# laurentbartholdi/SpaSM.jl

Measured on AMD Instinct MI355X. Metric: Schur nnz reduced/sec (GF(p) echelonize), 1Mx1M CSR, higher is better.
Workload: dtype int32 (GF(p) balanced residues); 1 GPU; BASELINE config 3: 1000000x1000000 CSR, 20 nnz/row, p=65521, seed 0x5A5A0003, Schur round 0; rows_per_gpu=1000000, npiv=169473, nnz_out=522630694, parallelism=single GPU

## Files before the change

### spasm.jl_amd/csrc/engine.hip

```cpp
#include "common.hpp"
#include "kernels.hpp"
#include "stream.hpp"
#include "wlevel.hpp"
#include "greedy.hpp"
#include "dense.hpp"
#include "spmv.hpp"
#include "spgemm.hpp"
#include "reshape.hpp"
#include "trsolve.hpp"
#include "batch.hpp"
#include "blocks.hpp"
#include "solve_batch.hpp"
#include "solver.hpp"
#include <cstring>
#include <rocprim/device/device_scan.hpp>
#include <rocprim/device/device_radix_sort.hpp>
#include <rocprim/device/device_segmented_radix_sort.hpp>
#include <vector>
#include <memory>
#include <stdexcept>
#include <type_traits>
#include <algorithm>
#include <cstring>
#include <cstdlib>
// ... 1311 lines not shown
    {
        if (bigsc_m == m) return;
        const i64 per = std::max<i64>((i64)m, 1) * 13;
        bigsc_blocks = (int)std::max<i64>(1, std::min<i64>((i64)num_cu * 8, ((i64)2 << 30) / per));
        bigsc_m = m;
        const size_t nw = ((size_t)std::max(m, 1) + 31) / 32;
        sc_xdense.alloc((size_t)bigsc_blocks * (size_t)std::max(m, 1));
        sc_bitmap.alloc((size_t)bigsc_blocks * nw);
        sc_touched.alloc((size_t)bigsc_blocks * (size_t)std::max(m, 1));
        sc_xdense.zero(s);
        sc_bitmap.zero(s);
    }
    void warm_scatter()
    {
        ensure_streams();
        ensure_big_scatter(stream);
        ScatterArgs a;
        memset(&a, 0, sizeof a);
        StreamArgs sa;
        memset(&sa, 0, sizeof sa);
        const int nhash = F.small ? kNumHashClasses : kNumHashClasses - 1;
        for (int c = 0; c < nhash; c++) {
            const size_t lds = scatter_lds_bytes(kClasses[c], F.small);
            if (F.small) launch_scatter_class<true>(c, a, 0, lds, stream);
            else launch_scatter_class<false>(c, a, 0, lds, stream);
        }
        for (int c = 0; c < std::min(nhash, kNumStreamClasses); c++) {
            const size_t lds = stream_lds_bytes(stream_logt(c), stream_tpr(c), stream_wpb(c));
            const StreamMode mode = stream_mode(use_w ? wbase + wcap : 0);
            if (F.small) launch_stream_class<true>(c, sa, 0, num_cu, lds, stream, mode);
            else launch_stream_class<false>(c, sa, 0, num_cu, lds, stream, mode);
        }
    }

    void run_scatter(const DevMat &M, const int *rows, int nrows)
    {
        const int4 *recs = Lpool.p;
        S.n = nrows;
        S.m = m;
        nlaunch = 0;
        if (nrows == 0) return;
        int nhash = F.small ? kNumHashClasses : kNumHashClasses - 1;
        const bool streaming = use_w && !force_lists && !want_idx;
        BinArgs b;
        b.nrows = nrows;
        b.bound = bound.p;
        b.Llen = Llen.p;
        for (int c = 0; c < NCLASS; c++) b.cap[c] = -1;
        for (int c = 0; c < nhash; c++) b.cap[c] = kClasses[c].cap;
        b.lazy_terms = zp_lazy_terms(F);
        b.class_count = class_count.p;
        b.class_list = class_list.p;
        b.rows = rows;
        b.start = M.start.p;
        b.len = M.len.p;
        b.orig = M.orig.p;
        b.Lstart = Lstart.p;
        b.sstart = sstart.p;
        b.pmask = pmask.p;
        b.sflag = sflag.p;
        b.stream_classes = streaming ? std::min(nhash, kNumStreamClasses) : 0;
        b.Sorig = S.orig.p;
        b.fixcnt = fixcnt.p;
        b.desc = class_desc.p;
        hipLaunchKernelGGL(k_bin, dim3(cdiv(nrows, 1024)), dim3(256), 0, stream, b);
        HIPCHK(hipGetLastError());

        ScatterArgs a;
        a.ent = M.ent.p;
        a.qinv_r = qinv_r.p;
        a.uhdr = uhdr.p;
        a.UPN = UPN.p;
        a.Lpool = recs;
        a.Sent = S.ent.p;
        a.Slen = S.len.p;
        a.Slead = S.lead.p;
        a.ctr = ctr.p;
        a.F = F;
        {
            const char *dbg = getenv("SPASM_DBG");
            a.dbg = dbg ? atoi(dbg) : 0;
        }
        a.stamps = nullptr;
#ifdef SPASM_STAMPS
        stamps.ensure(NCLASS * 2 * NSTAMP);
        HIPCHK(hipMemsetAsync(stamps.p, 0, NCLASS * 2 * NSTAMP * sizeof(u64d), stream));
        a.stamps = stamps.p;
#endif
        StreamArgs sa;
        sa.ent = M.ent.p;
        sa.qinv_r = qinv_r.p;
        sa.UPN = UPN.p;
        sa.Lpool = recs;
        sa.Sent = S.ent.p;
        sa.Slen = S.len.p;
        sa.Slead = S.lead.p;
        sa.ctr = ctr.p;
        sa.F = F;
        sa.dbg = a.dbg;
        sa.stamps = a.stamps;
        sa.fixbuf = fixbuf.p;
        sa.fixcnt = fixcnt.p;
        nhash_used = nhash;
        const int first_side = 6;
        const bool use_side = !class_timing && (nhash > first_side || streaming);
        if (use_side) {
            ensure_streams();
            HIPCHK(hipEventRecord(ev_fork, stream));
            HIPCHK(hipStreamWaitEvent(side, ev_fork, 0));
        }
        auto mark = [&](int cls_id, hipStream_t s) {
            if (!class_timing || nlaunch >= NCLASS) return;
            HIPCHK(hipEventRecord(ev_cls[nlaunch], s));
            launch_cls[nlaunch++] = cls_id;
        };
        auto launch_class = [&](int c, hipStream_t s) {
            mark(c, s);
            a.cls = c;
            a.class_count = class_count.p + c;
            a.desc = class_desc.p + (size_t)c * nrows;
            const size_t lds = scatter_lds_bytes(kClasses[c], F.small);
            int per_cu = (int)std::min<size_t>(32 / kClasses[c].wpb, (160 * 1024) / lds);
            if (per_cu < 1) per_cu = 1;
            const int rows_per_block = kClasses[c].tpr == 64 ? kClasses[c].wpb : 1;
            const int grid = std::max(1, std::min(cdiv(nrows, rows_per_block), num_cu * per_cu));
            if (F.small) launch_scatter_class<true>(c, a, grid, lds, s);
            else launch_scatter_class<false>(c, a, grid, lds, s);
        };
        auto launch_stream_cls = [&](int c, hipStream_t s) {
            if (!streaming || c >= kNumStreamClasses) return;
            mark(NSTREAM0 + c, s);
            sa.cls = NSTREAM0 + c;
            sa.class_count = class_count.p + NSTREAM0 + c;
            sa.desc = class_desc.p + (size_t)(NSTREAM0 + c) * nrows;
            sa.redo_count = class_count.p + c;
            sa.redo_desc = class_desc.p + (size_t)c * nrows;
            const size_t lds = stream_lds_bytes(stream_logt(c), stream_tpr(c), stream_wpb(c));
            if (F.small) launch_stream_class<true>(c, sa, nrows, num_cu, lds, s, smode);
            else launch_stream_class<false>(c, sa, nrows, num_cu, lds, s, smode);
        };
        auto launch_stream_fix = [&](hipStream_t s) {
            if (!streaming) return;
            mark(NCLASS - 1, s);
            StreamFixArgs fa;
            fa.nrows = nrows;
            fa.fixcnt = fixcnt.p;
            fa.fixbuf = fixbuf.p;
            fa.sstart = sstart.p;
            fa.Sent = S.ent.p;
            fa.Slen = S.len.p;
            fa.Slead = S.lead.p;
            fa.ctr = ctr.p;
            fa.F = F;
            hipLaunchKernelGGL(k_stream_fix, dim3(cdiv(nrows, 64)), dim3(256), 0, s, fa);
            HIPCHK(hipGetLastError());
        };
        auto launch_big = [&](hipStream_t s) {
            ensure_big_scatter(s);
            mark(NHASHMAX - 1, s);
            BigScatterArgs bb;
            bb.s = a;
            bb.s.cls = NHASHMAX - 1;
            bb.s.class_count = class_count.p + (NHASHMAX - 1);
            bb.s.desc = class_desc.p + (size_t)(NHASHMAX - 1) * nrows;
            bb.m = std::max(m, 1);
            bb.nwords = (std::max(m, 1) + 31) / 32;
            bb.xdense = sc_xdense.p;
            bb.bitmap = sc_bitmap.p;
            bb.touched = sc_touched.p;
            hipLaunchKernelGGL(k_scatter_big, dim3(bigsc_blocks), dim3(256), 0, s, bb);
            HIPCHK(hipGetLastError());
        };
        if (use_side && streaming) {
            const int lanes = n_lanes();
            for (int l = 1; l < lanes; l++) HIPCHK(hipStreamWaitEvent(lane_s[l], ev_fork, 0));
            const int ntwin = n_twins();
            for (int c = nhash - 1; c >= 0; c--) {
                const int l = (nhash - 1 - c) % lanes;
                hipStream_t lane = l ? lane_s[l] : stream;
                launch_stream_cls(c, lane);
                HIPCHK(hipEventRecord(ev_cls_done[c], lane));
                const int t = (nhash - 1 - c) % ntwin;
                hipStream_t tw = t ? twin_s[t - 1] : side;
                HIPCHK(hipStreamWaitEvent(tw, ev_cls_done[c], 0));
                launch_class(c, tw);
            }
            for (int l = 1; l < lanes; l++) {
                HIPCHK(hipEventRecord(lane_ev[l], lane_s[l]));
                HIPCHK(hipStreamWaitEvent(stream, lane_ev[l], 0));
            }
            for (int t = 0; t < ntwin - 1; t++) {
                HIPCHK(hipEventRecord(twin_ev[t], twin_s[t]));
                HIPCHK(hipStreamWaitEvent(stream, twin_ev[t], 0));
            }
            launch_stream_fix(stream);
            launch_big(side);
            HIPCHK(hipEventRecord(ev_join, side));
            HIPCHK(hipStreamWaitEvent(stream, ev_join, 0));
        } else if (use_side) {
            for (int c = nhash - 1; c >= first_side; c--) launch_class(c, side);
            launch_big(side);
            HIPCHK(hipEventRecord(ev_join, side));
            for (int c = 0; c < first_side; c++) launch_class(c, stream);
            HIPCHK(hipStreamWaitEvent(stream, ev_join, 0));
        } else {
            for (int c = nhash - 1; c >= 0; c--) launch_stream_cls(c, stream);
            launch_stream_fix(stream);
            for (int c = 0; c < nhash; c++) launch_class(c, stream);
            launch_big(stream);
            if (class_timing) HIPCHK(hipEventRecord(ev_cls[nlaunch], stream));
        }
        hipLaunchKernelGGL(k_scatter_mark_failed, dim3(cdiv(nrows, 256)), dim3(256), 0, stream, nrows, Llen.p, S.len.p, S.lead.p);
        HIPCHK(hipGetLastError());
        HIPCHK(hipMemcpyAsync(S.start.p, sstart.p, ((size_t)nrows + 1) * sizeof(i64d), hipMemcpyDeviceToDevice, stream));
    }

    void fetch_counters()
    {
        hctr = read_counters();
        int *cc = hclass_count;
        HIPCHK(hipMemcpyAsync(cc, class_count.p, NCLASS * sizeof(int), hipMemcpyDeviceToHost, stream));
        HIPCHK(hipStreamSynchronize(stream));
#ifdef SPASM_STAMPS
        {
            std::vector<u64d> h(NCLASS * 2 * NSTAMP);
            HIPCHK(hipMemcpy(h.data(), stamps.p, h.size() * sizeof(u64d), hipMemcpyDeviceToHost));
            static const char *names[NSTAMP] = {"prologue", "issue", "wait-loads", "own", "rounds", "remainder", "sweep", "-"};
            static const char *snames[NSTAMP] = {"top+own", "chunks", "next-req", "rowend", "reset", "rotate", "-", "-"};
            for (int c = NSTREAM0; c < NCLASS; c++) {
                const double waves = (double)h[(size_t)c * 2 * NSTAMP + NSTAMP];
                if (waves == 0) continue;
                fprintf(stderr, "[stamps] stream class %d rows %d waves %.0f: cycles per wave:", c - NSTREAM0, cc[c], waves);
                for (int i = 0; i < 6; i++) fprintf(stderr, " %s=%.0f", snames[i], (double)h[(size_t)c * 2 * NSTAMP + i] / waves);
                fprintf(stderr, "\n");
            }
            for (int c = 0; c < NHASHMAX; c++) {
                const double waves = (double)h[(size_t)c * 2 * NSTAMP + NSTAMP];
                if (waves == 0) continue;
                fprintf(stderr, "[stamps] class %d rows %d waves %.0f: cycles per wave:", c, cc[c], waves);
                for (int i = 0; i < 7; i++) fprintf(stderr, " %s=%.0f", names[i], (double)h[(size_t)c * 2 * NSTAMP + i] / waves);
                fprintf(stderr, "\n");
            }
        }
#endif
        if (hctr.lpool_overflow) throw EngineError("multiplier pool exhausted");
        if (hctr.scatter_overflow) throw EngineError("a hash table of the scatter kernel filled up (internal bound violated)");
    }
};

void upload_csr_strided(const struct spasm_csr *A, int row_lo, int row_hi, int stride, DevMat &M, hipStream_t s);

void upload_csr(const struct spasm_csr *A, int row_lo, int row_hi, DevMat &M, hipStream_t s)
{
    const int n = row_hi - row_lo;
    const i64 base = A->p[row_lo];
    const i64 nnz = A->p[row_hi] - base;
    M.n = n;
    M.m = A->m;
    M.start.ensure((size_t)n + 1);
    M.len.ensure((size_t)n + 1);
    M.lead.ensure((size_t)n + 1);
    M.orig.ensure((size_t)n + 1);
    M.ent.ensure((size_t)nnz + 1);
    DevBuf<i64d> dp;
    DevBuf<int> dj, dx;
    dp.alloc((size_t)n + 1);
    dj.alloc((size_t)nnz + 1);
    dx.alloc((size_t)nnz + 1);
    std::vector<i64d> hp((size_t)n + 1);
    for (int i = 0; i <= n; i++) hp[(size_t)i] = A->p[row_lo + i] - base;
    HIPCHK(hipMemcpyAsync(dp.p, hp.data(), ((size_t)n + 1) * sizeof(i64d), hipMemcpyHostToDevice, s));
    if (nnz > 0) {
        HIPCHK(hipMemcpyAsync(dj.p, A->j + base, (size_t)nnz * sizeof(int), hipMemcpyHostToDevice, s));
        if (A->x) HIPCHK(hipMemcpyAsync(dx.p, A->x + base, (size_t)nnz * sizeof(int), hipMemcpyHostToDevice, s));
        hipLaunchKernelGGL(k_pack_entries, dim3(std::min<i64>(cdiv(nnz, 256), 65536)), dim3(256), 0, s, (i64d)nnz, zp_field_make(A->field->p), dj.p,
                           A->x ? dx.p : nullptr, M.ent.p);
        HIPCHK(hipGetLastError());
    }
    if (n > 0) {
        hipLaunchKernelGGL(k_pack_rows, dim3(cdiv(n, 256)), dim3(256), 0, s, n, row_lo, 1, dp.p, M.start.p, M.len.p, M.orig.p);
        HIPCHK(hipGetLastError());
        constexpr int TEAM = 8;
        if (A->x) hipLaunchKernelGGL((k_drop_zeros<TEAM>), dim3(cdiv((i64)n * TEAM, 256)), dim3(256), 0, s, n, M.start.p, M.len.p, M.ent.p);
        hipLaunchKernelGGL((k_row_lead<TEAM>), dim3(cdiv((i64)n * TEAM, 256)), dim3(256), 0, s, n, M.start.p, M.len.p, M.ent.p, M.lead.p);
        HIPCHK(hipGetLastError());
    }
    HIPCHK(hipStreamSynchronize(s));
}

void upload_csr_strided(const struct spasm_csr *A, int row_lo, int row_hi, int stride, DevMat &M, hipStream_t s)
{
    if (stride <= 1) { upload_csr(A, row_lo, row_hi, M, s); return; }
    const int n = row_hi > row_lo ? (row_hi - row_lo + stride - 1) / stride : 0;
    std::vector<i64d> hp((size_t)n + 1, 0);
    for (int i = 0; i < n; i++) { const int g = row_lo + i * stride; hp[(size_t)i + 1] = hp[(size_t)i] + (A->p[g + 1] - A->p[g]); }
    const i64 nnz = hp[(size_t)n];
    std::vector<int> hj((size_t)nnz + 1), hx((size_t)nnz + 1);
    for (int i = 0; i < n; i++) {
        const int g = row_lo + i * stride;
        const i64 len = A->p[g + 1] - A->p[g];
        memcpy(hj.data() + hp[(size_t)i], A->j + A->p[g], sizeof(int) * (size_t)len);
        if (A->x) memcpy(hx.data() + hp[(size_t)i], A->x + A->p[g], sizeof(int) * (size_t)len);
    }
    M.n = n;
    M.m = A->m;
    M.start.ensure((size_t)n + 1);
    M.len.ensure((size_t)n + 1);
// ... 7615 lines not shown
```

### spasm.jl_amd/csrc/stream.hpp

```cpp
#pragma once
#include "kernels.hpp"

struct StreamArgs {
    const int *class_count;
    const RowDesc *desc;
    const int2 *ent;
    const int *qinv_r;
    const int2 *UPN;
    const int4 *Lpool;
    int2 *Sent;
    int *Slen;
    int *Slead;
    RoundCounters *ctr;
    int cls;
    int *redo_count;
    RowDesc *redo_desc;
    int2 *fixbuf;
    int *fixcnt;
    u64d *stamps;
    int dbg;
    ZpField F;
};

constexpr int SLCAP = 64;
constexpr int SFIX = 64;

__host__ __device__ constexpr size_t stream_row_bytes(int logt) { return ((size_t)7 << logt) + 64 + (size_t)SFIX * 8 + (size_t)SLCAP * 16; }
__host__ __device__ constexpr size_t stream_lds_bytes(int logt, int tpr, int wpb) { return tpr == 64 ? stream_row_bytes(logt) * (size_t)wpb : stream_row_bytes(logt); }

__device__ __forceinline__ void stream_fix_push(int *s_nfix, int2 *fix, int fcap, int owner_pos, int pos, int v)
{
    const int i = atomicAdd(s_nfix, 1);
    if (i < fcap) fix[i] = make_int2((int)(((unsigned)owner_pos << 14) | (unsigned)pos), v);
}

constexpr unsigned STREAM_K1 = 0x9E3779u, STREAM_K2 = 0x85EBCBu, STREAM_K3 = 0xC2B2AFu;

template <bool SMALL> __device__ __forceinline__ int stream_mul(const ZpField &F, int nm, int y);
template <> __device__ __forceinline__ int stream_mul<true>(const ZpField &F, int nm, int y) { return acc_reduce_short<true>(F, __mul24(nm, y)); }
template <> __device__ __forceinline__ int stream_mul<false>(const ZpField &F, int nm, int y) { return zp_mul(F, nm, y); }

__device__ __forceinline__ u64d stream_load_fresh(const u64d *p) { return __hip_atomic_load(p, __ATOMIC_RELAXED, __HIP_MEMORY_SCOPE_AGENT); }

template <int FCAP>
__device__ __forceinline__ int stream_fixup(const ZpField F, const int2 *fix, int nfix, int *scratch, u64d *row, int E, int *lead)
{
    constexpr int HC = 2 * FCAP;
    const int lane = threadIdx.x & 63;
    int *holes = scratch, *tailflag = scratch + HC, *lowh = scratch + 2 * HC, *livet = scratch + 3 * HC;
    for (int b = 0; b < nfix; b += 64) {
        const int f = b + lane;
        if (f < nfix) {
            const int2 e = fix[f];
            const int po = (int)((unsigned)e.x >> 14);
            holes[f] = e.x & 0x3fff;
            u64d *p = row + po;
            u64d cur = stream_load_fresh(p);
            for (;;) {
                const int nv = zp_add(F, (int)(cur >> 32), e.y);
                const u64d want = ((u64d)(unsigned)nv << 32) | (cur & 0xffffffffull);
                const u64d old = atomicCAS(p, cur, want);
                if (old == cur) break;
                cur = old;
            }
        }
    }
    int nh = nfix, nz = 0;
    for (int b = 0; b < nfix; b += 64) {
        const int f = b + lane;
        int po = -1;
        bool z = false;
        if (f < nfix) {
            po = (int)((unsigned)fix[f].x >> 14);
            z = (int)(stream_load_fresh(row + po) >> 32) == 0;
        }
        u64d mz = __ballot(z);
        while (mz) {
            const int l = __ffsll((long long)mz) - 1;
            mz &= mz - 1;
            const int pz = __shfl(po, l);
            bool dup = false;
            for (int i = nfix + lane; i < nh; i += 64) dup |= holes[i] == pz;
            if (__ballot(dup) == 0) {
                if (lane == 0) holes[nh] = pz;
                nh++;
                nz++;
            }
        }
    }
    const int n_out = E - nh;
    for (int i = lane; i < nh; i += 64) tailflag[i] = 0;
    for (int i = lane; i < nh; i += 64) {
        const int hp = holes[i];
        if (hp >= n_out) tailflag[hp - n_out] = 1;
    }
    int nlow = 0, nlive = 0;
    for (int b = 0; b < nh; b += 64) {
        const int i = b + lane;
        const bool in = i < nh;
        const int hp = in ? holes[i] : INT_MAX;
        const bool low = in && hp < n_out;
        const u64d ml = __ballot(low);
        if (low) lowh[nlow + __popcll(ml & lanemask_lt())] = hp;
        nlow += __popcll(ml);
        const bool live = in && tailflag[i] == 0;
        const u64d mv = __ballot(live);
        if (live) livet[nlive + __popcll(mv & lanemask_lt())] = n_out + i;
        nlive += __popcll(mv);
    }
    for (int i = lane; i < nlow; i += 64) row[lowh[i]] = stream_load_fresh(row + livet[i]);
    if (nz > 0) {
        asm volatile("s_waitcnt vmcnt(0)" ::: "memory");
        int mn = INT_MAX;
        for (int i = lane; i < n_out; i += 64) mn = min(mn, (int)(unsigned)stream_load_fresh(row + i));
        *lead = wave_min_i32(mn);
    }
    return n_out;
}


__device__ __forceinline__ int stream_desc_load(const RowDesc *p) { return ((const int *)p)[(threadIdx.x & 63) % 12]; }
__device__ __forceinline__ RowDesc stream_desc_unpack(int v)
{
    RowDesc d;
    const unsigned w0 = __builtin_amdgcn_readlane(v, 0), w1 = __builtin_amdgcn_readlane(v, 1), w2 = __builtin_amdgcn_readlane(v, 2),
                   w3 = __builtin_amdgcn_readlane(v, 3), w4 = __builtin_amdgcn_readlane(v, 4), w5 = __builtin_amdgcn_readlane(v, 5),
                   w10 = __builtin_amdgcn_readlane(v, 10), w11 = __builtin_amdgcn_readlane(v, 11);
    d.ent_start = (i64d)(((u64d)w1 << 32) | w0);
    d.l_start = (i64d)(((u64d)w3 << 32) | w2);
    d.s_start = (i64d)(((u64d)w5 << 32) | w4);
    d.len = __builtin_amdgcn_readlane(v, 6);
    d.llen = __builtin_amdgcn_readlane(v, 7);
    d.t = __builtin_amdgcn_readlane(v, 8);
    d.bound = __builtin_amdgcn_readlane(v, 9);
    d.pmask = (long long)(((u64d)w11 << 32) | w10);
    return d;
}

__device__ __forceinline__ unsigned stream_mul24(int c, unsigned k)
{
    unsigned x;
    asm("v_mul_u32_u24 %0, %1, %2" : "=v"(x) : "v"(c), "s"(k));
    return x;
}

template <int LOGT> struct StreamTabs {
    static constexpr int WORDS = (1 << LOGT) + (1 << (LOGT - 1)) + (1 << (LOGT - 2));
    unsigned *t1;
    __device__ __forceinline__ void bind(unsigned char *p) { t1 = (unsigned *)p; }
    template <int LV> __device__ __forceinline__ unsigned want(int c, int pos1, unsigned &slot) const
    {
        constexpr int L = LOGT - LV;
        constexpr unsigned K = LV == 0 ? STREAM_K1 : (LV == 1 ? STREAM_K2 : STREAM_K3);
        constexpr unsigned BASE = LV == 0 ? 0u : (LV == 1 ? (1u << LOGT) : (1u << LOGT) + (1u << (LOGT - 1)));
        const unsigned x = stream_mul24(c, K);
        slot = BASE + __builtin_amdgcn_ubfe(x, 24 - L, L);
        return (x << 14) | (unsigned)pos1;
    }
};

template <int LOGT, int N>
__device__ __forceinline__ void stream_insert_n(const StreamTabs<LOGT> &tb, const int (&c)[N], const int (&pos1)[N], unsigned (&old)[N], unsigned (&left)[N])
{
    unsigned w1[N], s1[N];
#pragma unroll
    for (int j = 0; j < N; j++) w1[j] = tb.template want<0>(c[j], pos1[j], s1[j]);
#pragma unroll
    for (int j = 0; j < N; j++) old[j] = atomicCAS(&tb.t1[s1[j]], 0u, w1[j]);
#pragma unroll
    for (int j = 0; j < N; j++) left[j] = old[j] == 0 ? 0u : old[j] ^ w1[j];
#pragma unroll
    for (int j = 0; j < N; j++) {
        if (left[j] >= 0x4000u) {
            unsigned s2;
            const unsigned w2 = tb.template want<1>(c[j], pos1[j], s2);
            const unsigned o2 = atomicCAS(&tb.t1[s2], 0u, w2);
            old[j] = o2;
            left[j] = o2 == 0 ? 0u : o2 ^ w2;
        }
    }
#pragma unroll
    for (int j = 0; j < N; j++) {
        if (left[j] >= 0x4000u) {
            unsigned s3;
            const unsigned w3 = tb.template want<2>(c[j], pos1[j], s3);
            const unsigned o3 = atomicCAS(&tb.t1[s3], 0u, w3);
            old[j] = o3;
            left[j] = o3 == 0 ? 0u : o3 ^ w3;
        }
    }
}
__device__ __forceinline__ unsigned stream_outcome(unsigned left) { return left == 0 ? 0u : (left < 0x4000u ? 1u : 2u); }
template <int LOGT>
__device__ __forceinline__ unsigned stream_insert(const StreamTabs<LOGT> &tb, int c, int pos1, unsigned &old)
{
    const int cc[1] = {c}, pp[1] = {pos1};
    unsigned oo[1], rr[1];
    stream_insert_n<LOGT, 1>(tb, cc, pp, oo, rr);
    old = oo[0];
    return stream_outcome(rr[0]);
}

__device__ __forceinline__ void stream_report(unsigned res, unsigned old, bool prim, int c, int v, int pos1, int *misc, int2 *fix, int fcap, int4 *lst)
{
    if (!prim || res == 0) return;
    if (res == 1) stream_fix_push(misc, fix, fcap, (int)(old & 0x3fffu) - 1, pos1 - 1, v);
    else {
        const int i = atomicAdd(misc + 1, 1);
        if (i < SLCAP) lst[i] = make_int4(c, v, pos1 - 1, 0);
    }
}


struct WPlanArgs {
    int nrows;
    const i64d *rstart;
    const int *rlen;
    const int2 *ent;
    const unsigned *pbits;
    const int4 *wcol;
    int4 *Lpool;
    u64d lpool_cap;
    u64d *pool_ctr;
    int npool;
    int2 *upn;
    unsigned own_base;
    u64d own_cap;
    u64d *own_ctr;
    i64d *Lstart;
    int *Llen;
    i64d *bound;
    long long *pmask;
    int *sflag;
    int free_cols;
    int max_bound;
    int wave_row_bound;
    int *overflow_list;
    int *overflow_count;
    RoundCounters *ctr;
    ZpField F;
    int chunk_log;
};

template <int TEAM, int TPB, bool SEGP>
__global__ __launch_bounds__(TPB) void k_wplan(WPlanArgs a)
{
    constexpr int TEAMS = TPB / TEAM;
    constexpr u64d RBLK = 64, OBLK = 256;
    const int tl = threadIdx.x % TEAM;
    const int team = threadIdx.x / TEAM;
    const ZpField F = a.F;
    const int CL = a.chunk_log, CH = 1 << CL;
    u64d rpos = 0, rend = 0, opos = 0, oend = 0;
    auto take = [&](u64d &pos, u64d &end, u64d need, u64d blk, u64d *ctr, u64d cap) -> u64d {
        if (pos + need > end) {
            const u64d n = need > blk ? need : blk;
            u64d b = 0;
            if (tl == 0) b = pool_alloc(ctr, cap, n, a.npool);
            b = __shfl(b, 0, TEAM);
            if (b == ~0ull) return ~0ull;
            pos = b;
            end = b + n;
        }
        const u64d r = pos;
        pos += need;
        return r;
    };
    auto is_piv = [&](int c) -> bool { return (a.pbits[(unsigned)c >> 5] >> (c & 31)) & 1u; };
// ... 382 lines not shown
        if (my_chunks > D) {
            SegRegs sr = {0, 0, 0};
            if constexpr (SEG) sr = seg_regs(rec, ll);
            for (int g0 = D; g0 < my_chunks; g0 += Q) {
                ring_t e[Q];
                int em[Q];
#pragma unroll
                for (int q = 0; q < Q; q++) {
                    const int g = min(g0 + q, my_chunks - 1);
                    em[q] = 0;
                    if constexpr (SEG) {
                        unsigned boff;
                        seg_locate(sr, E, g, boff, em[q]);
                        e[q] = seg_load(boff);
                    } else {
                        e[q] = ring_load((unsigned)__builtin_amdgcn_readlane(rec.z, g), __builtin_amdgcn_readlane(rec.w, g));
                    }
                }
                do_group(e, em, g0, my_chunks - g0);
            }
        }
        STAMP(1);
        request(rec_n, next_chunks, next_live, dn.llen, dn.bound);
        STAMP(2);
        mylead = wave_min_i32(mylead);
        int lead_out = mylead;
        if (!WAVE_ROW) {
            if (lane == 0) mrow[4 + wave] = mylead;
            lds_barrier();
#pragma unroll
            for (int w2 = 0; w2 < WPB; w2++) lead_out = min(lead_out, mrow[4 + w2]);
        }
        if constexpr (BLOOM) {
            const int nsus = __builtin_amdgcn_readfirstlane(((lds_vint *)mrow)[1]);
            if (nsus != 0 && nsus <= SLCAP) {
                auto scan = [&](bool owners) {
                    for (int g0 = 0; g0 < my_chunks; g0 += 8) {
                        int2 e[8];
                        int ps[8], nm[8];
                        bool ok[8];
#pragma unroll
                        for (int u = 0; u < 8; u++) {
                            const int g = min(g0 + u, my_chunks - 1);
                            const int clen = __builtin_amdgcn_readlane(rec.w, g);
                            e[u] = a.UPN[(size_t)(unsigned)__builtin_amdgcn_readlane(rec.z, g) + (unsigned)min(lane, clen - 1)];
                            ps[u] = (int)((unsigned)__builtin_amdgcn_readlane(rec.x, g) >> 16) + lane;
                            nm[u] = -__builtin_amdgcn_readlane(rec.y, g);
                            ok[u] = g0 + u < my_chunks && lane < clen;
                        }
                        for (int i = 0; i < nsus; i++) {
                            const int4 sp = lst[i];
                            if (owners && !(sp.w != INT_MAX && sp.w > sp.z)) continue;
#pragma unroll
                            for (int u = 0; u < 8; u++) {
                                if (ok[u] && e[u].x == sp.x && ps[u] != sp.z) {
                                    if (!owners) atomicMin(&lst[i].w, ps[u]);
                                    else {
                                        bool plain = true;
                                        for (int j = 0; j < nsus; j++) plain = plain && lst[j].z != ps[u];
                                        if (plain) stream_fix_push(mrow, fix, FCAP, sp.z, ps[u], stream_mul<SMALL>(F, nm[u], e[u].y));
                                    }
                                }
                            }
                        }
                    }
                };
                scan(false);
                if (!WAVE_ROW) lds_barrier();
                bool any_owner = false;
                for (int i = 0; i < nsus; i++) {
                    const int4 sp = lst[i];
                    if (sp.w == INT_MAX) continue;
                    if (sp.w < sp.z) { if ((WAVE_ROW || wave == 0) && lane == 0) stream_fix_push(mrow, fix, FCAP, sp.w, sp.z, sp.y); }
                    else any_owner = true;
                }
                if (any_owner) {
                    scan(true);
                    if (!WAVE_ROW) lds_barrier();
                }
            }
        }
        if (WAVE_ROW || wave == 0) {
            bool redo = false;
            const int nlist = __builtin_amdgcn_readfirstlane(((lds_vint *)mrow)[1]);
            redo = nlist > SLCAP;
            if (!BLOOM && nlist != 0 && !redo) {
                for (int b = 0; b < nlist; b += 64) {
                    const int i = b + lane;
                    int4 me = make_int4(-1, 0, -1, 0);
                    if (i < nlist) me = lst[i];
                    int owner = -1;
                    for (int j = 0; j < nlist; j++) {
                        const int4 o = lst[j];
                        if (j < i && owner < 0 && o.x == me.x && o.z != me.z) owner = o.z;
                    }
                    if (owner >= 0) stream_fix_push(mrow, fix, FCAP, owner, me.z, me.y);
                }
            }
            const int nfix = SCATTER_DBG(a, 4) ? 0 : __builtin_amdgcn_readfirstlane(((lds_vint *)mrow)[0]);
            redo = redo || nfix > FCAP;
            if (redo) {
                if (lane == 0) {
                    const int at = atomicAdd(a.redo_count, 1);
                    a.redo_desc[at] = d;
                }
                c_redo += 1;
            } else {
                if (lane < nfix) a.fixbuf[(size_t)t_cur * SFIX + lane] = fix[lane];
                if (lane == 0) {
                    a.Slen[t_cur] = E;
                    a.Slead[t_cur] = E > 0 ? lead_out : INT_MAX;
                    if (nfix) a.fixcnt[t_cur] = nfix;
                }
                c_nnz += (u64d)E;
                c_rows += E > 0;
                c_ent += (u64d)E;
                c_seg += 1 + (u64d)row_chunks(d);
            }
        }
        STAMP(3);
        for (int s = rtid * 4; s < StreamTabs<LOGT>::WORDS; s += TPR * 4) *(int4 *)(tb.t1 + s) = make_int4(0, 0, 0, 0);
        if (WAVE_ROW) {
            if (lane < 2) mrow[lane] = 0;
            __builtin_amdgcn_wave_barrier();
        } else {
            par ^= 1;
            if (rtid < 8) misc[par * 8 + rtid] = rtid >= 4 ? INT_MAX : 0;
            lds_barrier();
        }
        STAMP(4);
        d = dn;
        dn = dnn;
        dnn = stream_desc_unpack(d3_reg);
        rec = rec_n; rec_n = rec_nn;
        STAMP(5);
    }
#ifdef SPASM_STAMPS
    if (lane == 0 && a.stamps) {
        for (int i = 0; i < NSTAMP; i++) atomicAdd(&a.stamps[(size_t)a.cls * 2 * NSTAMP + i], st_sum[i]);
        atomicAdd(&a.stamps[(size_t)a.cls * 2 * NSTAMP + NSTAMP], 1ull);
    }
#endif
    if (lane == 0 && (WAVE_ROW || wave == 0)) {
        if (c_nnz) atomicAdd(&ctr_shard(a.ctr)->nnz_out, c_nnz);
        if (c_rows) atomicAdd(&ctr_shard(a.ctr)->nonempty_out, c_rows);
        if (c_redo) atomicAdd(&ctr_shard(a.ctr)->stream_redo, c_redo);
        if (c_ent | c_seg) {
            atomicAdd(&ctr_shard(a.ctr)->class_ent[a.cls], c_ent);
            atomicAdd(&ctr_shard(a.ctr)->class_seg[a.cls], c_seg);
        }
    }
}

struct StreamFixArgs {
    int nrows;
    const int *fixcnt;
    const int2 *fixbuf;
    const i64d *sstart;
    int2 *Sent;
    int *Slen;
    int *Slead;
    RoundCounters *ctr;
    ZpField F;
};

__global__ __launch_bounds__(256) void k_stream_fix(StreamFixArgs a)
{
    __shared__ int s_scratch[4][8 * SFIX];
    const int lane = threadIdx.x & 63, wave = threadIdx.x >> 6;
    const int t0 = (blockIdx.x * 4 + wave) * 16;
    if (t0 >= a.nrows) return;
    const int mine = (lane < 16 && t0 + lane < a.nrows) ? a.fixcnt[t0 + lane] : 0;
    u64d m = __ballot(mine > 0);
    u64d holes = 0;
    int emptied = 0, merged = 0;
    while (m) {
        const int l = __ffsll((long long)m) - 1;
        m &= m - 1;
        const int t = t0 + l;
        const int n = __builtin_amdgcn_readlane(mine, l);
        const int E = a.Slen[t];
        int lead = a.Slead[t];
        const int n_out = stream_fixup<SFIX>(a.F, a.fixbuf + (size_t)t * SFIX, n, s_scratch[wave], (u64d *)(a.Sent + a.sstart[t]), E, &lead);
        if (lane == 0) {
            a.Slen[t] = n_out;
            a.Slead[t] = n_out > 0 ? lead : INT_MAX;
        }
        holes += (u64d)(E - n_out);
        emptied += (n_out == 0 && E > 0);
        merged += n;
    }
    if (lane == 0 && merged) {
        atomicAdd(&ctr_shard(a.ctr)->nnz_out, (u64d)0 - holes);
        if (emptied) atomicAdd(&ctr_shard(a.ctr)->nonempty_out, -emptied);
        atomicAdd(&ctr_shard(a.ctr)->stream_fix, merged);
    }
}
```

Measured before the change: 184.1 billion nnz/s.

## Restructure stream fixup kernel into 16-lane teams with wave-wide batched merges

The fixup kernel now covers 64 rows per wave instead of 16. For rows with at most 16 fixes, all fix entries are merged wave-wide in one batch, with an LDS hash claim table that serializes conflicting writes to the same slot. Each 16-lane team then compacts its own rows, using a DPP row-min reduction. Rows with more fixes still go through the old whole-wave path, and the lead-min scan is unrolled four loads deep. This trades much more code complexity and LDS use, plus retry loops on hash collisions, for less serialization across lanes in a kernel that may only be a small part of the round.

```diff
diff --git a/spasm.jl_amd/csrc/engine.hip b/spasm.jl_amd/csrc/engine.hip
--- a/spasm.jl_amd/csrc/engine.hip
+++ b/spasm.jl_amd/csrc/engine.hip
@@ -1487,7 +1487,7 @@
             fa.Slead = S.lead.p;
             fa.ctr = ctr.p;
             fa.F = F;
-            hipLaunchKernelGGL(k_stream_fix, dim3(cdiv(nrows, 64)), dim3(256), 0, s, fa);
+            hipLaunchKernelGGL(k_stream_fix, dim3(cdiv(nrows, 4 * SFIX_SLOTS)), dim3(256), 0, s, fa);
             HIPCHK(hipGetLastError());
         };
         auto launch_big = [&](hipStream_t s) {
diff --git a/spasm.jl_amd/csrc/stream.hpp b/spasm.jl_amd/csrc/stream.hpp
--- a/spasm.jl_amd/csrc/stream.hpp
+++ b/spasm.jl_amd/csrc/stream.hpp
@@ -42,6 +42,19 @@
 
 __device__ __forceinline__ u64d stream_load_fresh(const u64d *p) { return __hip_atomic_load(p, __ATOMIC_RELAXED, __HIP_MEMORY_SCOPE_AGENT); }
 
+template <int N> __device__ __forceinline__ int stream_row_lead(const u64d *row, int n, int l)
+{
+    int mn = INT_MAX;
+    for (int i0 = l; i0 < n; i0 += 4 * N) {
+        u64d v[4];
+#pragma unroll
+        for (int u = 0; u < 4; u++) v[u] = stream_load_fresh(row + min(i0 + u * N, n - 1));
+#pragma unroll
+        for (int u = 0; u < 4; u++) mn = min(mn, (int)(unsigned)v[u]);
+    }
+    return mn;
+}
+
 template <int FCAP>
 __device__ __forceinline__ int stream_fixup(const ZpField F, const int2 *fix, int nfix, int *scratch, u64d *row, int E, int *lead)
 {
@@ -111,9 +124,7 @@
     for (int i = lane; i < nlow; i += 64) row[lowh[i]] = stream_load_fresh(row + livet[i]);
     if (nz > 0) {
         asm volatile("s_waitcnt vmcnt(0)" ::: "memory");
-        int mn = INT_MAX;
-        for (int i = lane; i < n_out; i += 64) mn = min(mn, (int)(unsigned)stream_load_fresh(row + i));
-        *lead = wave_min_i32(mn);
+        *lead = wave_min_i32(stream_row_lead<64>(row, n_out, lane));
     }
     return n_out;
 }
@@ -802,6 +813,73 @@
     }
 }
 
+__device__ __forceinline__ int row16_min_i32(int x)
+{
+    x = min(x, __builtin_amdgcn_update_dpp(x, x, 0x128, 0xf, 0xf, false));
+    x = min(x, __builtin_amdgcn_update_dpp(x, x, 0x124, 0xf, 0xf, false));
+    x = min(x, __builtin_amdgcn_update_dpp(x, x, 0x122, 0xf, 0xf, false));
+    x = min(x, __builtin_amdgcn_update_dpp(x, x, 0x121, 0xf, 0xf, false));
+    return x;
+}
+
+template <int TEAM>
+__device__ __forceinline__ int stream_fixup_team(const int2 *fix, int nfix, int *scratch, u64d *row, int E, int *lead)
+{
+    static_assert(TEAM == 16, "a team is a DPP row");
+    constexpr int HC = 2 * TEAM;
+    const int tl = threadIdx.x & (TEAM - 1);
+    const u64d below = (1ull << tl) - 1ull;
+    int *holes = scratch, *tailflag = scratch + HC, *lowh = scratch + 2 * HC, *livet = scratch + 3 * HC;
+    int po = -1;
+    bool z = false;
+    if (tl < nfix) {
+        const int ex = fix[tl].x;
+        po = (int)((unsigned)ex >> 14);
+        holes[tl] = ex & 0x3fff;
+        z = (int)(stream_load_fresh(row + po) >> 32) == 0;
+    }
+    int nh = nfix, nz = 0;
+    u64d mz = team_ballot<TEAM>(z);
+    while (mz) {
+        const int l = __ffsll((long long)mz) - 1;
+        mz &= mz - 1;
+        const int pz = __shfl(po, l, TEAM);
+        bool dup = false;
+        for (int i = nfix + tl; i < nh; i += TEAM) dup |= holes[i] == pz;
+        if (team_ballot<TEAM>(dup) == 0) {
+            if (tl == 0) holes[nh] = pz;
+            nh++;
+            nz++;
+        }
+    }
+    const int n_out = E - nh;
+    for (int i = tl; i < nh; i += TEAM) tailflag[i] = 0;
+    for (int i = tl; i < nh; i += TEAM) {
+        const int hp = holes[i];
+        if (hp >= n_out) tailflag[hp - n_out] = 1;
+    }
+    int nlow = 0, nlive = 0;
+    for (int b = 0; b < nh; b += TEAM) {
+        const int i = b + tl;
+        const bool in = i < nh;
+        const int hp = in ? holes[i] : INT_MAX;
+        const bool low = in && hp < n_out;
+        const u64d ml = team_ballot<TEAM>(low);
+        if (low) lowh[nlow + __popcll(ml & below)] = hp;
+        nlow += __popcll(ml);
+        const bool live = in && tailflag[i] == 0;
+        const u64d mv = team_ballot<TEAM>(live);
+        if (live) livet[nlive + __popcll(mv & below)] = n_out + i;
+        nlive += __popcll(mv);
+    }
+    for (int i = tl; i < nlow; i += TEAM) row[lowh[i]] = stream_load_fresh(row + livet[i]);
+    if (nz > 0) {
+        asm volatile("s_waitcnt vmcnt(0)" ::: "memory");
+        *lead = row16_min_i32(stream_row_lead<TEAM>(row, n_out, tl));
+    }
+    return n_out;
+}
+
 struct StreamFixArgs {
     int nrows;
     const int *fixcnt;
@@ -814,32 +892,127 @@
     ZpField F;
 };
 
+constexpr int SFIX_TEAM = 16;
+constexpr int SFIX_SLOTS = 64;
+constexpr int SFIX_CLAIM = 512;
+static_assert(SFIX_CLAIM == 1 << 9, "the hash of k_stream_fix keeps nine bits");
+
 __global__ __launch_bounds__(256) void k_stream_fix(StreamFixArgs a)
 {
+    static_assert(8 * SFIX >= (64 / SFIX_TEAM) * 8 * SFIX_TEAM, "the teams' scratch lies in the wave's");
     __shared__ int s_scratch[4][8 * SFIX];
+    __shared__ int s_incl[4][64];
+    __shared__ __attribute__((aligned(16))) unsigned s_claim[4][SFIX_CLAIM];
     const int lane = threadIdx.x & 63, wave = threadIdx.x >> 6;
-    const int t0 = (blockIdx.x * 4 + wave) * 16;
+    const int t0 = (blockIdx.x * 4 + wave) * SFIX_SLOTS;
     if (t0 >= a.nrows) return;
-    const int mine = (lane < 16 && t0 + lane < a.nrows) ? a.fixcnt[t0 + lane] : 0;
-    u64d m = __ballot(mine > 0);
+    const ZpField F = a.F;
+    int cnt = 0, E = 0, lead = INT_MAX;
+    i64d ss = 0;
+    if (t0 + lane < a.nrows) {
+        cnt = a.fixcnt[t0 + lane];
+        E = a.Slen[t0 + lane];
+        lead = a.Slead[t0 + lane];
+        ss = a.sstart[t0 + lane];
+    }
+    if (__ballot(cnt > 0) == 0) return;
+    const int cnt_team = cnt <= SFIX_TEAM ? cnt : 0;
+    int total;
+    const int incl = team_incl_scan<64>(cnt_team, total);
+    int *const s_in = s_incl[wave];
+    unsigned *const claim = s_claim[wave];
+    s_in[lane] = incl;
+    __builtin_amdgcn_wave_barrier();
+    for (int b = 0; b < total; b += 64) {
+        const int f = b + lane;
+        int r = 0;
+#pragma unroll
+        for (int step = 32; step > 0; step >>= 1)
+            if (s_in[r + step - 1] <= f) r += step;
+        const int first = r > 0 ? s_in[r - 1] : 0;
+        const i64d rs = __shfl(ss, r);
+        bool pend = f < total;
+        int val = 0;
+        unsigned key = 0;
+        u64d *p = nullptr;
+        if (pend) {
+            const int2 e = a.fixbuf[(size_t)(t0 + r) * SFIX + (f - first)];
+            const unsigned po = (unsigned)e.x >> 14;
+            val = e.y;
+            key = (((unsigned)r << 14) | po) + 1u;
+            p = (u64d *)(a.Sent + rs) + po;
+        }
+        while (__ballot(pend) != 0) {
+            for (int q = lane * 4; q < SFIX_CLAIM; q += 256) *(int4 *)(claim + q) = make_int4(0, 0, 0, 0);
+            __builtin_amdgcn_wave_barrier();
+            bool win = false;
+            if (pend) {
+                unsigned h = (key * 0x9E3779B1u) >> 23;
+                for (;;) {
+                    const unsigned old = atomicCAS(&claim[h], 0u, key);
+                    win = old == 0u;
+                    if (win || old == key) break;
+                    h = (h + 1) & (SFIX_CLAIM - 1);
+                }
+            }
+            if (win) {
+                const u64d cur = stream_load_fresh(p);
+                const int nv = zp_add(F, (int)(cur >> 32), val);
+                *p = ((u64d)(unsigned)nv << 32) | (cur & 0xffffffffull);
+                pend = false;
+            }
+            asm volatile("s_waitcnt vmcnt(0)" ::: "memory");
+        }
+    }
+    __builtin_amdgcn_fence(__ATOMIC_ACQ_REL, "workgroup");
     u64d holes = 0;
     int emptied = 0, merged = 0;
+    {
+        const int tl = lane & (SFIX_TEAM - 1), tbase = lane & ~(SFIX_TEAM - 1);
+        int *const tscratch = s_scratch[wave] + (lane / SFIX_TEAM) * (8 * SFIX_TEAM);
+        u64d m = team_ballot<SFIX_TEAM>(cnt_team > 0);
+        while (m) {
+            const int src = tbase + __ffsll((long long)m) - 1;
+            m &= m - 1;
+            const int n = __shfl(cnt, src);
+            const int Er = __shfl(E, src);
+            int ld = __shfl(lead, src);
+            const i64d rs = __shfl(ss, src);
+            const int n_out = stream_fixup_team<SFIX_TEAM>(a.fixbuf + (size_t)(t0 + src) * SFIX, n, tscratch, (u64d *)(a.Sent + rs), Er, &ld);
+            if (tl == 0) {
+                a.Slen[t0 + src] = n_out;
+                a.Slead[t0 + src] = n_out > 0 ? ld : INT_MAX;
+                holes += (u64d)(Er - n_out);
+                emptied += (n_out == 0 && Er > 0);
+                merged += n;
+            }
+        }
+    }
+    __builtin_amdgcn_wave_barrier();
+    u64d m = __ballot(cnt > SFIX_TEAM);
     while (m) {
         const int l = __ffsll((long long)m) - 1;
         m &= m - 1;
         const int t = t0 + l;
-        const int n = __builtin_amdgcn_readlane(mine, l);
-        const int E = a.Slen[t];
-        int lead = a.Slead[t];
-        const int n_out = stream_fixup<SFIX>(a.F, a.fixbuf + (size_t)t * SFIX, n, s_scratch[wave], (u64d *)(a.Sent + a.sstart[t]), E, &lead);
+        const int n = __builtin_amdgcn_readlane(cnt, l);
+        const int Er = __builtin_amdgcn_readlane(E, l);
+        int ld = __builtin_amdgcn_readlane(lead, l);
+        const i64d rs = __shfl(ss, l);
+        const int n_out = stream_fixup<SFIX>(F, a.fixbuf + (size_t)t * SFIX, n, s_scratch[wave], (u64d *)(a.Sent + rs), Er, &ld);
         if (lane == 0) {
             a.Slen[t] = n_out;
-            a.Slead[t] = n_out > 0 ? lead : INT_MAX;
-        }
-        holes += (u64d)(E - n_out);
-        emptied += (n_out == 0 && E > 0);
-        merged += n;
-    }
+            a.Slead[t] = n_out > 0 ? ld : INT_MAX;
+            holes += (u64d)(Er - n_out);
+            emptied += (n_out == 0 && Er > 0);
+            merged += n;
+        }
+    }
+    holes += __shfl_xor(holes, 16);
+    emptied += __shfl_xor(emptied, 16);
+    merged += __shfl_xor(merged, 16);
+    holes += __shfl_xor(holes, 32);
+    emptied += __shfl_xor(emptied, 32);
+    merged += __shfl_xor(merged, 32);
     if (lane == 0 && merged) {
         atomicAdd(&ctr_shard(a.ctr)->nnz_out, (u64d)0 - holes);
         if (emptied) atomicAdd(&ctr_shard(a.ctr)->nonempty_out, -emptied);
```

After: 186.3 billion nnz/s (median of 3 runs). Within noise of the previous version (+1.2%).
